# kureta/ddsp-pytorch

Hardware: AMD Instinct MI355X
Metric: audio samples/sec/GPU + %HBM-roofline, 16kHz/100-harmonic/batch512 (higher is better)
Workload: dtype f32

## Files before the change

ddsp-pytorch_amd/csrc/ddsp_osc.hip:

```cpp
#include <hip/hip_runtime.h>
#include <stdint.h>

#include <atomic>

#include "ddsp_hip.h"
#include "ddsp_internal.h"
#include "ddsp_osc_common.h"

using namespace ddsp_osc;

namespace {

template <int K, int MODE, bool POW2, int KL = K, int NS = 1, bool QREUSE = false>
__device__ __forceinline__ void walk_fast(const OscParams &p, FrameState<K> &st, int b, int t, int j, bool active,
                                          int i0, float L0, float L1, int n_beg, int n_end)
{
    extern __shared__ float ystage[];
    const float i0f = (float)i0;
    float *yframe = p.y + ((long)b * p.T + t) * p.R;
    float lam = 0.0f, dlam = 0.0f;
    if (POW2) {
        float w0s;
        upsample_weights(p.scale, t * p.R + n_beg, i0f, w0s, lam);
        dlam = (t == 0 && n_beg == 0) ? 0.0f : p.scale;
    }
#define DDSP_STAGE_END() __builtin_amdgcn_sched_barrier(0)
    constexpr bool QKEEP = QREUSE && (MODE == MODE_SYNTH) && POW2 && NS == 1;
    float qk[QKEEP ? KL : 1];
    auto one_step = [&](int n, const bool fresh) {
        float w0[NS], w1[NS];
#pragma unroll
        for (int e = 0; e < NS; ++e) {
            if (POW2) {
                w1[e] = lam;
                w0[e] = 1.0f - lam;
                lam += dlam;
            } else {
                upsample_weights(p.scale, t * p.R + n + e, i0f, w0[e], w1[e]);
            }
        }
// ... 452 lines not shown
    const double occupancy = K >= 20 ? 1.10 : (K >= 15 ? 1.03 : 1.0);
    const double waves = (double)(frames << logG) / 64.0;
    const double fill = waves >= 2048.0 ? 1.0 : (waves < 1.0 ? 1.0 : waves) / 2048.0;
    return waste * shared * occupancy / fill;
}

std::atomic<int> g_forced_k{0};
std::atomic<int> g_path{0};

bool pick_tiling(int H, long frames, Tiling *out)
{
    double best = 1e30;
    bool found = false;
    const int forced = g_forced_k.load(std::memory_order_relaxed);
    for (int K : kKs) {
        if (forced && K != forced) continue;
        const int lanes = (H + K - 1) / K;
        int logG = 0;
        while ((1 << logG) < lanes) ++logG;
        if (logG > 6) continue;
        const double cost = tiling_cost(H, K, logG, frames);
        if (cost < best) {
            best = cost;
            out->K = K;
            out->logG = logG;
            found = true;
        }
    }
    return found;
}

size_t frame_scratch_bytes(int B, int T, int H)
{
    const size_t n = (size_t)B * T * H;
    return 2 * align256(n * sizeof(float)) + align256(n * sizeof(double)) + align256(sup_elems(B, T, H) * sizeof(double)) + 256;
}

bool setup_params(OscParams &p, void *scratch, int B, int T, int H, int hop, int sample_rate)
{
    Tiling tl;
    if (!pick_tiling(H, (long)B * T, &tl)) return false;
    const size_t n = (size_t)B * T * H;
    char *base = (char *)scratch;
    p.w = (float *)base;
    p.amp = (float *)(base + align256(n * sizeof(float)));
    p.loc = (double *)(base + 2 * align256(n * sizeof(float)));
    p.sup = (double *)((char *)p.loc + align256(n * sizeof(double)));
    p.redo_flag = (int *)((char *)p.sup + align256(sup_elems(B, T, H) * sizeof(double)));
    p.B = B; p.T = T; p.H = H; p.R = hop;
    p.K = tl.K;
    p.logG = tl.logG;
    p.NSB = (T + (256 >> tl.logG) - 1) / (256 >> tl.logG);
    p.scale = (float)(1.0 / (double)hop);
    p.nyquist = (float)(sample_rate / 2);
    p.sr = (float)sample_rate;
    p.pow2 = ((hop & (hop - 1)) == 0 && hop >= 2 && (long)T * hop <= (1L << 23)) ? 1 : 0;
    p.stage_out = (p.pow2 && hop >= 64 && tl.logG >= 2 && tl.logG <= 4) ? 1 : 0;
    return true;
}

}

extern "C" int ddsp_osc_set_tiling(int harmonics_per_lane)
{
    if (harmonics_per_lane != 0) {
        if (!ddsp_hooks_on()) return DDSP_EPERM;
        bool known = false;
        for (int K : kKs) known = known || (K == harmonics_per_lane);
// ... 82 lines not shown
```

ddsp-pytorch_amd/csrc/ddsp_osc_chunk.hip:

```cpp
#include <hip/hip_runtime.h>
#include <stdint.h>

#include <atomic>
#include <mutex>
#include <stdlib.h>
#include <vector>

#include "ddsp_hip.h"
#include "ddsp_internal.h"
#include "ddsp_osc_common.h"
#include "ddsp_osc_plan.h"

#include <stddef.h>

using namespace ddsp_osc;

namespace {

#ifndef DDSP_TURN_EVERY
#define DDSP_TURN_EVERY 8
#endif
constexpr int kRow = 256 + 4;
constexpr float kReuseMaxInc = 4.8f;

#define DDSP_STAGE_END() __builtin_amdgcn_sched_barrier(0)

__device__ __forceinline__ void segment_lambda(const OscParams &p, int n, bool clamp0, float &lam, float &dlam)
{
    lam = clamp0 ? 0.0f : (float)(2 * n + 1) * p.inv2R;
    dlam = clamp0 ? 0.0f : 2.0f * p.inv2R;
}

__device__ __forceinline__ int wave_slot()
{
    return __builtin_amdgcn_s_getreg((4 << 0) | (0 << 6) | (3 << 11));
}
__device__ __forceinline__ void take_turn(int slot, int nres, int shift)
{
    const unsigned epoch = (unsigned)(__builtin_amdgcn_s_memrealtime() >> shift);
    const unsigned turn = epoch + (unsigned)slot;
    switch (nres >= 3 ? turn % 3u : (nres == 2 ? (turn & 1u) : 0u)) {
        case 0: __builtin_amdgcn_s_setprio(0); break;
        case 1: __builtin_amdgcn_s_setprio(1); break;
        default: __builtin_amdgcn_s_setprio(2); break;
    }
}

__device__ __forceinline__ float ldf(const float *base, unsigned idx)
{
    return *reinterpret_cast<const float *>(reinterpret_cast<const char *>(base) + (size_t)(idx * 4u));
}
__device__ __forceinline__ double ldd(const double *base, unsigned idx)
{
    return *reinterpret_cast<const double *>(reinterpret_cast<const char *>(base) + (size_t)(idx * 8u));
}

struct ChunkArgs {
    OscParams p;
    PlanTable t;
};
__device__ __forceinline__ const PlanTable *plan_table()
{
    return reinterpret_cast<const PlanTable *>((const char *)__builtin_amdgcn_kernarg_segment_ptr() + offsetof(ChunkArgs, t));
}

template <int K>
struct ParentTable {
    int v[kPlanMaxK];
    constexpr ParentTable() : v()
    {
        for (int d = 0; d < kPlanMaxK; ++d) v[d] = derived_parent(K, d);
    }
};
#define DDSP_PARENT(K, d) (par.v[d])

template <int K, int KR>
struct ChunkState {
    double acc[KR];
    float x0[KR], x1[KR];
    float a1[K], da[K];
};

struct Task {
    int wt, rb, c;
    int b, j;
    bool active;
    int i, i_end;
    int s, n;
};

__device__ __forceinline__ Task decode_task(const OscParams &p, int wt)
{
    Task k;
    k.wt = wt;
    k.rb = wt / p.NC;
    k.c = wt - k.rb * p.NC;
    const int lane = threadIdx.x & 63;
    k.j = lane & ((1 << p.logG) - 1);
    k.b = k.rb * (64 >> p.logG) + (lane >> p.logG);
    k.active = k.b < p.B;
    if (!k.active) k.b = p.B - 1;
    k.i = k.c * p.Lc;
    k.i_end = min(k.i + p.Lc, p.T * p.R);
    k.s = (k.i + (p.R >> 1)) >> p.lgR;
    k.n = (k.i + (p.R >> 1)) & (p.R - 1);
    return k;
}

__device__ __forceinline__ void segment_rows(int s, int T, int &r0, int &r1)
{
    r0 = s == 0 ? 0 : s - 1;
    r1 = s == 0 ? min(1, T - 1) : min(s, T - 1);
}

template <int K, int KR, int KLR, int NS, int QMODE>
__device__ __forceinline__ void walk_synth(const OscParams &p, ChunkState<K, KR> &st, const float (&fac)[K - KR + 1], float *ystage,
                                           float *yrow, int j, bool active, int i_abs, int n_beg, int n_end, bool clamp0, float L0,
                                           float L1, int slot)
{
    constexpr int KLD = KR < K ? class_derived(K, KLR) : 0;
    constexpr int KL = KLR + KLD;
#define DDSP_SLOT(m) ((m) < KLR ? (m) : KR + ((m) - KLR))
    constexpr ParentTable<K> par;
    const int G = 1 << p.logG, per = 32 >> p.logG;
    float lam, dlam;
    segment_lambda(p, n_beg, clamp0, lam, dlam);
    float mal = 1.0f - lam;
    float *ycol = ystage + threadIdx.x;
    const float *yblk = ystage + (threadIdx.x & ~(G - 1));
    static_assert(QMODE == 0 || (QMODE == 1 && NS == 1) || (QMODE == 2 && NS == 2), "quotient reuse: across iterations or inside a pair");
    float qk[QMODE == 1 ? KL : 1];
    constexpr int RUN = DDSP_TURN_EVERY < NS ? NS : DDSP_TURN_EVERY;
    for (int nb = n_beg; nb < n_end; nb += RUN) {
    take_turn(slot, p.nres, p.turn_shift);
    for (int n = nb; n < nb + RUN; n += NS) {
        float w0[NS], w1[NS];
        w1[0] = lam;
        w0[0] = mal;
#pragma unroll
        for (int e = 1; e < NS; ++e) {
            w1[e] = w1[e - 1] + dlam;
            w0[e] = w0[e - 1] - dlam;
        }
        float v[NS][KL];
        DDSP_STAGE_END();
#pragma unroll
        for (int e = 0; e < NS; ++e)
#pragma unroll
            for (int m = 0; m < KLR; ++m) v[e][m] = w1[e] * st.x1[m];
        DDSP_STAGE_END();
#pragma unroll
        for (int e = 0; e < NS; ++e)
#pragma unroll
            for (int m = 0; m < KLR; ++m) v[e][m] = __fmaf_rn(w0[e], st.x0[m], v[e][m]);
        DDSP_STAGE_END();
        double d[NS][KLR];
#pragma unroll
        for (int e = 0; e < NS; ++e)
#pragma unroll
            for (int m = 0; m < KLR; ++m) d[e][m] = (double)v[e][m];
        DDSP_STAGE_END();
#pragma unroll
        for (int e = 0; e < NS; ++e)
#pragma unroll
            for (int m = 0; m < KLR; ++m) {
                st.acc[m] += d[e][m];
                d[e][m] = st.acc[m];
// ... 155 lines not shown
    float lam, dlam;
    segment_lambda(p, n_beg, clamp0, lam, dlam);
    float mal = 1.0f - lam;
    for (int nb = n_beg; nb < n_end; nb += 16) {
    take_turn(slot, p.nres, p.turn_shift);
    for (int n = nb; n < nb + 16; ++n) {
        const float w1 = lam, w0 = mal;
        lam += dlam;
        mal -= dlam;
        float v[K];
        DDSP_STAGE_END();
#pragma unroll
        for (int m = 0; m < K; ++m) v[m] = w1 * x1[m];
        DDSP_STAGE_END();
#pragma unroll
        for (int m = 0; m < K; ++m) v[m] = __fmaf_rn(w0, x0[m], v[m]);
        DDSP_STAGE_END();
        double d[K];
#pragma unroll
        for (int m = 0; m < K; ++m) d[m] = (double)v[m];
        DDSP_STAGE_END();
#pragma unroll
        for (int m = 0; m < K; ++m) acc[m] += d[m];
        DDSP_STAGE_END();
    }
    }
}

__device__ __forceinline__ int group_max(int v, int logG)
{
    for (int o = 1; o < (1 << logG); o <<= 1) v = max(v, __shfl_xor(v, o));
    return v;
}

template <int K, int KR>
__global__ void __launch_bounds__(256, K <= 13 ? 3 : 1) osc_chunk_totals_kernel(ChunkArgs args)
{
    const OscParams &p = args.p;
    const int wt = blockIdx.x * 4 + __builtin_amdgcn_readfirstlane((int)(threadIdx.x >> 6));
    if (wt >= p.RB * p.NC) return;
    Task k = decode_task(p, wt);
    const int G = 1 << p.logG;
    const long rowbase = (long)k.b * p.T;
    const int i_beg = k.i;
    const int slot = wave_slot();
    int hs[K];
    {
        const PlanTable *tab = plan_table();
#pragma unroll
        for (int m = 0; m < K; ++m) hs[m] = tab->h[k.j * K + m];
    }
    int hmax = 0;

    auto make_row = [&](int r, float (&w)[KR]) {
        const float fb = p.f0[rowbase + r];
        const unsigned crow = ((unsigned)k.b * p.T + r) * p.H;
        float a0[K];
        float s = 0.0f;
#pragma unroll
        for (int m = 0; m < K; ++m) a0[m] = ldf(p.c, crow + min(hs[m], p.H - 1));
#pragma unroll
        for (int m = 0; m < K; ++m) {
            const int h = hs[m];
            const bool ok = h < p.H;
            const float hz = (float)(h + 1) * fb;
            a0[m] = (ok && !(hz > p.nyquist)) ? a0[m] : 0.0f;
            s += a0[m];
        }
        s = group_sum(s, p.logG);
        const float rs = 1.0f / s;
        const int seg_start = max(r * p.R - (p.R >> 1), 0);
        const bool own = k.active && seg_start >= i_beg && seg_start < k.i_end;
#pragma unroll
        for (int m = 0; m < K; ++m) {
            const int h = hs[m];
            const bool ok = h < p.H;
            const float wv = ok ? frame_increment(h, fb, p.sr) : 0.0f;
            if (m < KR) w[m < KR ? m : 0] = wv;
            const float amp = ok ? a0[m] * rs : 0.0f;
            if (amp != 0.0f) hmax = max(hmax, h + 1);
            if (ok && own) {
                p.w[crow + h] = wv;
                p.amp[crow + h] = amp;
            }
        }
    };

    float x0[KR], x1[KR];
    int r0, r1;
    segment_rows(k.s, p.T, r0, r1);
    make_row(r0, x0);
    make_row(r1, x1);
    double acc[KR];
#pragma unroll
    for (int m = 0; m < KR; ++m) acc[m] = 0.0;
    while (true) {
        const int n_end = min(p.R, k.n + (k.i_end - k.i));
        walk_totals<KR>(p, acc, x0, x1, k.n, n_end, k.s == 0, slot);
        k.i += n_end - k.n;
        if (k.i >= k.i_end) break;
        ++k.s; k.n = 0;
        if (k.s >= 2) {
#pragma unroll
            for (int m = 0; m < KR; ++m) x0[m] = x1[m];
            if (k.s <= p.T - 1) make_row(k.s, x1);
        }
    }
    hmax = group_max(hmax, p.logG);
    if (k.active) {
        double *cp = p.ctot + ((long)k.b * p.NC + k.c) * p.HC + k.j;
#pragma unroll
        for (int m = 0; m < KR; ++m)
            if (hs[m] < p.H) cp[m * G] = acc[m];
        if (k.j == 0) p.rlive[(long)k.b * p.NC + k.c] = hmax;
    }
}

__global__ void __launch_bounds__(512) osc_chunk_scan_kernel(OscParams p, int nscan_blocks, int Q)
{
    __shared__ double seg_tot[8][64];
    const int lane = threadIdx.x & 63, q = threadIdx.x >> 6;
    if (blockIdx.x == 0 && threadIdx.x == 0) {
        *p.redo_flag = 0;
        p.frame_flag[2] = 0;
    }
    if ((int)blockIdx.x < nscan_blocks) {
        const long ncol = (long)p.B * p.HC;
        const long idx = (long)blockIdx.x * 64 + lane;
        const bool live = idx < ncol && q < Q;
        const int b = live ? (int)(idx / p.HC) : 0, h = live ? (int)(idx - (long)b * p.HC) : 0;
        double *col = p.ctot + (long)b * p.NC * p.HC + h;
        const int per = (p.NC + Q - 1) / Q, c_beg = q * per, c_end = min(c_beg + per, p.NC);
        if (per <= 32) {
            double v[32];
            double tot = 0.0;
#pragma unroll
            for (int i = 0; i < 32; ++i) {
                v[i] = (live && c_beg + i < c_end) ? col[(long)(c_beg + i) * p.HC] : 0.0;
                tot += v[i];
            }
// ... 39 lines not shown
        return;
    }
    const long wv = (long)(blockIdx.x - nscan_blocks) * (blockDim.x >> 6) + q;
    const int c = (int)wv;
    if (c >= p.NC) return;
    const int Bpad = p.RB * (64 >> p.logG);
    int *out = p.perm + (long)c * Bpad;
    auto cls_of = [&](int ml) {
        if (ml < 0) return -1;
        int q = 0;
        while (q < 4 && ml <= p.cls_max[q]) ++q;
        return q;
    };
    int base[5], cnt[5] = {0, 0, 0, 0, 0};
    for (int b0 = 0; b0 < p.B; b0 += 64) {
        const int b = b0 + lane;
        const int cls = cls_of(b < p.B ? p.rlive[(long)b * p.NC + c] : -1);
        for (int q = 0; q < 5; ++q) cnt[q] += __popcll(__ballot(cls == q));
    }
    base[0] = 0;
    for (int q = 1; q < 5; ++q) base[q] = base[q - 1] + cnt[q - 1];
    for (int b0 = 0; b0 < p.B; b0 += 64) {
        const int b = b0 + lane;
        const int cls = cls_of(b < p.B ? p.rlive[(long)b * p.NC + c] : -1);
        for (int q = 0; q < 5; ++q) {
            const unsigned long long mask = __ballot(cls == q);
            if (cls == q) out[base[q] + __popcll(mask & ((1ull << lane) - 1ull))] = b;
            base[q] += __popcll(mask);
        }
    }
    for (int b = p.B + lane; b < Bpad; b += 64) out[b] = -1;
}

#ifdef DDSP_CHUNK_STAMPS
__device__ long g_stamps[16384 * 4];
extern "C" int ddsp_osc_read_stamps(long *host, int ntasks)
{
    return (int)hipMemcpyFromSymbol(host, HIP_SYMBOL(g_stamps), sizeof(long) * 4 * (size_t)(ntasks < 16384 ? ntasks : 16384));
}
#endif

#ifndef DDSP_CHUNK_INLINE_REPAIR
#define DDSP_CHUNK_INLINE_REPAIR 1
#endif
template <int K, int KR, bool EXACT>
__global__ void __launch_bounds__(256, (!EXACT && K <= 13) ? 3 : 1) osc_chunk_synth_kernel(ChunkArgs args)
{
    const OscParams &p = args.p;
    extern __shared__ float ystage[];
    constexpr int KD = K - KR;
    constexpr ParentTable<K> par;
    constexpr int KE = class_prefix(KR, 3), KQ = class_prefix(KR, 2), KH = class_prefix(KR, 1), KT = class_prefix(KR, 0);
    const int ntasks = p.RB * p.NC;
    const PlanTable *tab = plan_table();
    const int jj = (threadIdx.x & 63) & ((1 << p.logG) - 1);
    float fac[KD + 1];
#pragma unroll
    for (int d = 0; d < KD; ++d) fac[d] = (float)(1u << tab->shift[jj * K + KR + d]);
    fac[KD] = 1.0f;
    int wt = blockIdx.x * 4 + __builtin_amdgcn_readfirstlane((int)(threadIdx.x >> 6));
    if (EXACT && *p.redo_flag == 0) return;
    for (; wt < ntasks; wt += gridDim.x * 4) {
        if (EXACT && p.redo[wt] == 0) continue;
#ifdef DDSP_CHUNK_STAMPS
        const long stamp0 = wall_clock64();
#endif
        if (!EXACT && wt == 0 && (threadIdx.x & 63) == 0) clock_stamp(p.redo_flag, 0);
        bool exact = EXACT;
      for (;;) {
        Task k = decode_task(p, wt);
        {
            const int idx = k.rb * (64 >> p.logG) + ((threadIdx.x & 63) >> p.logG);
            const int b = p.perm[(long)k.c * (p.RB * (64 >> p.logG)) + idx];
            k.active = b >= 0;
            k.b = k.active ? b : p.perm[(long)k.c * (p.RB * (64 >> p.logG))];
        }
        const int G = 1 << p.logG;
        const long rowbase = (long)k.b * p.T;
        float *yrow = p.y + (long)k.b * p.T * p.R;
        ChunkState<K, KR> st;
        const int slot = exact ? 0 : wave_slot();
        bool bad = false;
        const unsigned cbase = ((unsigned)k.b * p.NC + k.c) * p.HC + k.j;
#pragma unroll
        for (int m = 0; m < KR; ++m) {
            const double v = ldd(p.ctot, cbase + (unsigned)(m * G));
            st.acc[m] = (tab->h[k.j * K + m] < p.H) ? v : 0.0;
            bad = bad || !(st.acc[m] >= 0.0);
        }
        int mlive = p.H;
        if (!exact) {
            mlive = p.rlive[(long)k.b * p.NC + k.c];
#pragma unroll
            for (int o = 32; o > 0; o >>= 1) mlive = max(mlive, __shfl_xor(mlive, o));
            mlive = __builtin_amdgcn_readfirstlane(mlive);
        }
        int r0, r1;
        segment_rows(k.s, p.T, r0, r1);
        float L0, L1;
        auto load_rows = [&](int ra, int rb2, bool first) {
            const unsigned o0 = ((unsigned)k.b * p.T + ra) * p.H, o1 = ((unsigned)k.b * p.T + rb2) * p.H;
            float t0[KR], t1[KR], u0[K], u1[K];
            int hs[K];
#pragma unroll
            for (int m = 0; m < K; ++m) hs[m] = tab->h[k.j * K + m];
#pragma unroll
            for (int m = 0; m < K; ++m) {
                const unsigned g = (unsigned)min(hs[m], p.H - 1);
                if (m < KR) {
                    t0[m < KR ? m : 0] = first ? ldf(p.w, o0 + g) : 0.0f;
                    t1[m < KR ? m : 0] = ldf(p.w, o1 + g);
                }
                u0[m] = first ? ldf(p.amp, o0 + g) : 0.0f;
                u1[m] = ldf(p.amp, o1 + g);
            }
#pragma unroll
            for (int m = 0; m < K; ++m) {
                const bool ok = hs[m] < p.H;
                if (m < KR) {
                    if (first) st.x0[m < KR ? m : 0] = ok ? t0[m < KR ? m : 0] : 0.0f;
                    st.x1[m < KR ? m : 0] = ok ? t1[m < KR ? m : 0] : 0.0f;
                }
                const float older = first ? (ok ? u0[m] : 0.0f) : st.a1[m];
                st.a1[m] = ok ? u1[m] : 0.0f;
                st.da[m] = st.a1[m] - older;
            }
            if (first) L0 = p.a[rowbase + ra]; else L0 = L1;
            L1 = p.a[rowbase + rb2];
        };
        load_rows(r0, r1, true);
#ifdef DDSP_CHUNK_STAMPS
        long stamp_walk = 0;
        if (DDSP_CHUNK_STAMPS == 2) {
            float chk = 0.0f;
#pragma unroll
            for (int m = 0; m < KR; ++m) chk += st.x1[m] + st.da[m];
            if (__any(chk == 123456.0f)) bad = true;
            stamp_walk = wall_clock64();
        }
#endif
        while (true) {
            const int n_end = min(p.R, k.n + (k.i_end - k.i));
            const bool clamp0 = k.s == 0;
            bool big = false;
#pragma unroll
            for (int m = 0; m < KR; ++m) {
                bad = bad || !(st.x0[m] >= 0.0f) || !(st.x1[m] >= 0.0f);
                big = big || !(st.x0[m] < kReuseMaxInc) || !(st.x1[m] < kReuseMaxInc);
            }
#pragma unroll
            for (int d = 0; d < KD; ++d)
                big = big || !(fac[d] * st.x0[DDSP_PARENT(K, d)] < kReuseMaxInc) || !(fac[d] * st.x1[DDSP_PARENT(K, d)] < kReuseMaxInc);
            if (exact) {
                walk_synth_exact<K, KR>(p, st, fac, yrow, k.j, k.active, k.i, k.n, n_end, clamp0, L0, L1);
            } else if (mlive <= p.cls_max[3] && KE < KQ) {
                walk_synth<K, KR, KE, 4, 0>(p, st, fac, ystage, yrow, k.j, k.active, k.i, k.n, n_end, clamp0, L0, L1, slot);
            } else if (mlive <= p.cls_max[2] && KQ < KH) {
                walk_synth<K, KR, KQ, 4, 0>(p, st, fac, ystage, yrow, k.j, k.active, k.i, k.n, n_end, clamp0, L0, L1, slot);
            } else if (mlive <= p.cls_max[1] && KH < KT) {
                walk_synth<K, KR, KH, 2, 0>(p, st, fac, ystage, yrow, k.j, k.active, k.i, k.n, n_end, clamp0, L0, L1, slot);
            } else if (mlive <= p.cls_max[0] && KT < KR) {
                walk_synth<K, KR, KT, 1, 0>(p, st, fac, ystage, yrow, k.j, k.active, k.i, k.n, n_end, clamp0, L0, L1, slot);
            } else if (!__any(big)) {
                walk_synth<K, KR, KR, 1, 1>(p, st, fac, ystage, yrow, k.j, k.active, k.i, k.n, n_end, clamp0, L0, L1, slot);
            } else {
                walk_synth<K, KR, KR, 1, 0>(p, st, fac, ystage, yrow, k.j, k.active, k.i, k.n, n_end, clamp0, L0, L1, slot);
            }
            k.i += n_end - k.n;
            if (k.i >= k.i_end) break;
            ++k.s; k.n = 0;
            if (k.s >= 2) {
#pragma unroll
                for (int m = 0; m < KR; ++m) st.x0[m] = st.x1[m];
                segment_rows(k.s, p.T, r0, r1);
                load_rows(r0, r1, false);
            }
        }
        if (!exact) {
#pragma unroll
            for (int m = 0; m < KR; ++m) bad = bad || !(st.acc[m] < (double)kFastPhaseLimit);
#pragma unroll
            for (int d = 0; d < KD; ++d) bad = bad || !((double)fac[d] * st.acc[DDSP_PARENT(K, d)] < (double)kFastPhaseLimit);
            const bool redo = __any(bad);
            if (DDSP_CHUNK_INLINE_REPAIR && redo) { exact = true; continue; }
            if ((threadIdx.x & 63) == 0) {
                p.redo[wt] = redo ? 1 : 0;
                if (redo) atomicOr(p.redo_flag, 1);
                if (wt == 0) clock_stamp(p.redo_flag, 1);
            }
#ifdef DDSP_CHUNK_STAMPS
            if ((threadIdx.x & 63) == 0 && wt < 16384) {
                g_stamps[wt * 4 + 0] = stamp0;
                g_stamps[wt * 4 + 1] = wall_clock64();
                g_stamps[wt * 4 + 2] = __builtin_amdgcn_s_getreg((4 << 0) | (0 << 6) | (31 << 11));
                g_stamps[wt * 4 + 3] = DDSP_CHUNK_STAMPS == 2 ? stamp_walk : (long)__builtin_amdgcn_s_getreg((20 << 0) | (0 << 6) | (31 << 11));
            }
#endif
        } else if (DDSP_CHUNK_INLINE_REPAIR && !EXACT && (threadIdx.x & 63) == 0) {
            p.redo[wt] = 0;
            if (wt == 0) clock_stamp(p.redo_flag, 1);
        }
        break;
      }
    }
}

struct Residency { int cus, wg_per_cu; };

template <int K, int KR>
hipError_t synth_residency(Residency *out)
{
    static std::mutex mu;
    static Residency cache[64] = {};
    int dev = 0;
    hipError_t e = hipGetDevice(&dev);
    if (e != hipSuccess) return e;
    dev &= 63;
    std::lock_guard<std::mutex> lk(mu);
    if (cache[dev].cus == 0) {
        int cus = 0, nb = 0;
        e = hipDeviceGetAttribute(&cus, hipDeviceAttributeMultiprocessorCount, dev);
        if (e != hipSuccess) return e;
        e = hipOccupancyMaxActiveBlocksPerMultiprocessor(&nb, osc_chunk_synth_kernel<K, KR, false>, 256, sizeof(float) * 32 * kRow);
        if (e != hipSuccess) return e;
        if (cus <= 0 || nb <= 0) return hipErrorInvalidValue;
        cache[dev].cus = cus;
        cache[dev].wg_per_cu = nb;
// ... 40 lines not shown
        long Lc = (N + nc - 1) / nc;
        Lc = (Lc + 31) & ~31L;
        if (Lc < R) Lc = R;
        if (Lc == lastLc) continue;
        lastLc = (int)Lc;
        const long NC = (N + Lc - 1) / Lc;
        const long wgs = (NC * RB + 3) / 4;
        const long per_cu = (wgs + cus - 1) / cus;
        const double alone = per_cu == 1 ? 1.9 : (per_cu == 2 ? 1.03 : 1.0);
        const double cost = (double)per_cu * alone * ((double)Lc + c0);
        if (cost < best) {
            best = cost;
            bestLc = (int)Lc;
            bestNC = (int)NC;
        }
        if (Lc == R) break;
    }
    (void)wg_per_cu;
    *Lc_out = bestLc;
    *NC_out = bestNC;
}

bool chunked_eligible(const OscParams &p)
{
    if (!(p.pow2 && p.R >= 64 && p.R <= 8192 && p.logG >= 2 && p.logG <= 4 && !p.live_in && !p.live_out && !p.dbg_phi &&
          (long)p.B * p.T * p.H < (1L << 29)))
        return false;
    const int gpw = 64 >> p.logG, rb = (p.B + gpw - 1) / gpw;
    return (long)p.B * 100 >= (long)rb * gpw * 88 || g_chunk_any_batch.load(std::memory_order_relaxed);
}

size_t chunk_scratch_bytes(int B, int T, int H)
{
    return frame_scratch_bytes(B, T, H) + 2 * align256((size_t)B * T * sizeof(int)) +
           align256((size_t)T * ((size_t)B + 16) * sizeof(int)) + 256;
}

template <int K>
hipError_t chunk_geometry(OscParams &p, Residency *res_out)
{
    Residency res;
    const SlotPlan &pl = slot_plan(p.H, K, 1 << p.logG);
    hipError_t e = pl.KD ? synth_residency<K, plan_roots(K)>(&res) : synth_residency<K, K>(&res);
    if (e != hipSuccess) return e;
    p.HC = pl.KD ? pl.KR << p.logG : p.H;
    for (int q = 0; q < 4; ++q) p.cls_max[q] = pl.cls_max[q];
    const int GPW = 64 >> p.logG;
    p.RB = (p.B + GPW - 1) / GPW;
    p.lgR = 0;
    while ((1 << p.lgR) < p.R) ++p.lgR;
    p.inv2R = 0.5f / (float)p.R;
    pick_chunks(p.T, p.R, p.RB, res.cus, res.wg_per_cu, &p.Lc, &p.NC);
    if (ddsp_hooks_on()) {
        const char *e = getenv("DDSP_OSC_CHUNK_LEN");
        const int v = e ? atoi(e) : 0;
        if (v >= p.R && v % 32 == 0) {
            p.Lc = v;
            p.NC = (int)(((long)p.T * p.R + v - 1) / v);
        }
    }
    p.nres = res.wg_per_cu < 3 ? (res.wg_per_cu < 1 ? 1 : res.wg_per_cu) : 3;
    {
        const double ticks = (double)p.Lc * (double)p.K * 5.6;
        int sh = 8;
        while (sh < 16 && (double)(1 << (sh + 1)) <= ticks / 6.0) ++sh;
        p.turn_shift = sh;
        if (ddsp_hooks_on()) {
            const char *e = getenv("DDSP_OSC_TURN_SHIFT");
            const int v = e ? atoi(e) : 0;
            if (v >= 6 && v <= 20) p.turn_shift = v;
        }
    }
    *res_out = res;
    return hipSuccess;
}

void carve_chunk_scratch(OscParams &p, void *scratch)
{
    const size_t n = (size_t)p.B * p.T * p.H;
    char *base = (char *)scratch;
    p.frame_flag = p.redo_flag;
    p.w = (float *)base;
    p.amp = (float *)(base + align256(n * sizeof(float)));
    p.ctot = (double *)(base + 2 * align256(n * sizeof(float)));
    p.rlive = (int *)(base + frame_scratch_bytes(p.B, p.T, p.H));
    p.perm = (int *)((char *)p.rlive + align256((size_t)p.B * p.NC * sizeof(int)));
    p.redo = (int *)((char *)p.perm + align256((size_t)p.NC * p.RB * (64 >> p.logG) * sizeof(int)));
    p.redo_flag = (int *)((char *)p.redo + align256((size_t)p.RB * p.NC * sizeof(int)));
}

template <int K, int KR>
hipError_t launch_plan(const OscParams &p, const SlotPlan &pl, hipStream_t s)
{
    ChunkArgs args;
    args.p = p;
    args.t = pl.t;
    const long tasks = (long)p.RB * p.NC;
    const unsigned grid = (unsigned)((tasks + 3) / 4);
    int slot = ddsp_prof::begin(ddsp_prof::TOTALS, s);
    hipLaunchKernelGGL((osc_chunk_totals_kernel<K, KR>), dim3(grid), dim3(256), 0, s, args);
    ddsp_prof::end(slot, s);
    slot = ddsp_prof::begin(ddsp_prof::SCAN, s);
    const long nscan_blocks = ((long)p.B * p.HC + 63) / 64;
    const int Q = p.NC > 128 ? 8 : (p.NC > 64 ? 4 : (p.NC > 32 ? 2 : 1));
    hipLaunchKernelGGL(osc_chunk_scan_kernel, dim3((unsigned)(nscan_blocks + (p.NC + Q - 1) / Q)), dim3(64 * Q), 0, s, p, (int)nscan_blocks, Q);
    ddsp_prof::end(slot, s);
    slot = ddsp_prof::begin(ddsp_prof::SYNTH, s);
    hipLaunchKernelGGL((osc_chunk_synth_kernel<K, KR, false>), dim3(grid), dim3(256), sizeof(float) * 32 * kRow, s, args);
    ddsp_prof::end(slot, s);
    if (!DDSP_CHUNK_INLINE_REPAIR) {
        const unsigned rgrid = grid < 256u ? grid : 256u;
        hipLaunchKernelGGL((osc_chunk_synth_kernel<K, KR, true>), dim3(rgrid), dim3(256), 0, s, args);
    }
    return hipGetLastError();
}

template <int K>
hipError_t launch_chunked(OscParams p, void *scratch, hipStream_t s)
{
    Residency res;
    hipError_t e = chunk_geometry<K>(p, &res);
    if (e != hipSuccess) return e;
    carve_chunk_scratch(p, scratch);
    const SlotPlan &pl = slot_plan(p.H, K, 1 << p.logG);
    return pl.KD ? launch_plan<K, plan_roots(K)>(p, pl, s) : launch_plan<K, K>(p, pl, s);
}

hipError_t chunk_geometry_k(OscParams &p, int *cus, int *wg_per_cu)
{
    Residency res = {};
    hipError_t e = hipErrorInvalidValue;
    switch (p.K) {
#define DDSP_CASE(KK) case KK: e = chunk_geometry<KK>(p, &res); break;
        DDSP_CASE(4) DDSP_CASE(8) DDSP_CASE(12) DDSP_CASE(13) DDSP_CASE(15) DDSP_CASE(16) DDSP_CASE(20) DDSP_CASE(23) DDSP_CASE(25)
#undef DDSP_CASE
        default: break;
    }
    *cus = res.cus;
    *wg_per_cu = res.wg_per_cu;
    return e;
}

const int *chunk_flag_words(OscParams p)
{
    int cus = 0, wgs = 0;
    if (chunk_geometry_k(p, &cus, &wgs) != hipSuccess) return p.redo_flag;
    carve_chunk_scratch(p, (void *)p.w);
    return p.redo_flag;
}

hipError_t launch_chunked_k(const OscParams &p, void *scratch, hipStream_t s)
{
    switch (p.K) {
#define DDSP_CASE(KK) case KK: return launch_chunked<KK>(p, scratch, s);
        DDSP_CASE(4) DDSP_CASE(8) DDSP_CASE(12) DDSP_CASE(13) DDSP_CASE(15) DDSP_CASE(16) DDSP_CASE(20) DDSP_CASE(23) DDSP_CASE(25)
#undef DDSP_CASE
// ... 6 lines not shown
```

ddsp-pytorch_amd/csrc/ddsp_osc_common.h:

```cpp
#pragma once
#include <hip/hip_runtime.h>
#include <stdint.h>

#include <atomic>

namespace ddsp_osc {


constexpr float kTwoPi32 = 6.2831854820251465f;
constexpr float kInvTwoPi32 = 0.15915493667125702f;
constexpr float kRevPerRad = 0.15915494309189535f;
constexpr float kFastPhaseLimit = 1.0e7f;
constexpr float kRoundMagic = 12582912.0f;
constexpr int kFrameScratchTag = 0x46524d45;

struct OscParams {
    const float *f0, *c, *a;
    float *y;
    float *w, *amp;
    double *loc;
    double *sup;
    int *redo_flag;
    const float *live_in;
    float *live_out;
    float *dbg_phi;
    const float *grad_y;
    float *part_c;
    float *part_a;
    float *grad_c, *grad_a;
    int B, T, H, R;
    int K;
    int logG;
    int NSB;
    int force_exact;
    int stage_out;
    int pow2;
    double *ctot;
    int *rlive;
    int *perm;
    int *redo;
    int *frame_flag;
    int Lc, NC, RB;
    int HC;
    int cls_max[4];
    int lgR;
    int nres;
    int turn_shift;
    float inv2R;
    float scale;
    float nyquist;
    float sr;
};

__device__ __forceinline__ unsigned xcd_block(unsigned bid, unsigned nblocks)
{
    const unsigned per = nblocks >> 3;
    if (per == 0 || bid >= (per << 3)) return bid;
    return (bid & 7u) * per + (bid >> 3);
}

__device__ __forceinline__ void clock_stamp(int *redo_flag, int which)
{
    unsigned long long *w = reinterpret_cast<unsigned long long *>(redo_flag + 16) + 2 * which;
    w[0] = __builtin_amdgcn_s_memtime();
    w[1] = __builtin_amdgcn_s_memrealtime();
}

template <int CTRL>
__device__ __forceinline__ float dpp_mov(float v)
// ... 99 lines not shown
```

ddsp-pytorch_amd/csrc/ddsp_osc_plan.h:

```cpp
#pragma once
#include <stdint.h>

#include <algorithm>
#include <set>
#include <vector>

namespace ddsp_osc {

constexpr int kPlanMaxLanes = 16, kPlanMaxK = 25, kPlanMaxSlots = kPlanMaxLanes * kPlanMaxK;
constexpr int kPlanParents = 7;
constexpr int kPlanMaxChildren = 3;
constexpr uint16_t kNoHarmonic = 0xffff;

constexpr int pick7(int i, int a, int b, int c, int d, int e, int f, int g)
{
    return i == 0 ? a : i == 1 ? b : i == 2 ? c : i == 3 ? d : i == 4 ? e : i == 5 ? f : i == 6 ? g : 0;
}
constexpr int slot_children(int K, int i)
{
    switch (K) {
        case 4: return pick7(i, 1, 0, 0, 0, 0, 0, 0);
        case 8: return pick7(i, 2, 1, 0, 0, 0, 0, 0);
        case 12: return pick7(i, 3, 2, 1, 0, 0, 0, 0);
        case 13: return pick7(i, 3, 2, 1, 0, 0, 0, 0);
        case 15: return pick7(i, 3, 2, 1, 1, 0, 0, 0);
        case 16: return pick7(i, 3, 2, 1, 1, 0, 0, 0);
        case 20: return pick7(i, 3, 2, 2, 1, 1, 0, 0);
        case 23: return pick7(i, 3, 2, 2, 1, 1, 1, 0);
        case 25: return pick7(i, 3, 2, 2, 1, 1, 1, 1);
        default: return 0;
    }
}
constexpr int plan_derived(int K)
// ... 123 lines not shown
    if (!s.place(0)) return false;

    pl.H = H; pl.K = K; pl.G = G; pl.KR = KR; pl.KD = KD;
    for (int i = 0; i < kPlanMaxSlots; ++i) { pl.t.h[i] = kNoHarmonic; pl.t.shift[i] = 0; }
    int derived = 0;
    for (int sz = kPlanMaxChildren + 1; sz >= 1; --sz) {
        std::vector<const Piece *> ps;
        for (const Piece &p : s.pieces)
            if (p.size_class == sz) ps.push_back(&p);
        std::sort(ps.begin(), ps.end(), [](const Piece *a, const Piece *b) { return a->members[0] < b->members[0]; });
        std::vector<int> idx;
        for (int i = 0; i < KR; ++i)
            if (1 + slot_children(K, i) == sz) idx.push_back(i);
        for (size_t n = 0; n < ps.size(); ++n) {
            const int i = idx[n / G], j = (int)(n % G);
            const std::vector<int> &mem = ps[n]->members;
            pl.t.h[j * K + i] = (uint16_t)(mem[0] - 1);
            for (size_t c = 1; c < mem.size(); ++c) {
                int d = 0;
                while (!(derived_parent(K, d) == i && derived_rank(K, d) == (int)c - 1)) ++d;
                int t = 0;
                while ((mem[0] << t) < mem[c]) ++t;
                pl.t.h[j * K + KR + d] = (uint16_t)(mem[c] - 1);
                pl.t.shift[j * K + KR + d] = (uint8_t)t;
                ++derived;
            }
        }
    }
    if (derived < 1) return false;
    plan_class_limits(pl);
    return true;
}

}
```

Baseline: 28.53 billion.

## Pack per-lane frame records contiguously and prefetch next row ahead of walks

Replaces the separate per-harmonic w and amp scratch arrays with one packed per-lane record of increments and amplitudes, written and read as float4 vectors. The synth kernel then loads rows with contiguous vector loads instead of scattered per-harmonic loads. The totals kernel now issues the next row's f0 and coefficient loads before walking the current segment so their latency overlaps compute, and the synth walk touches the next record early as a prefetch. Scratch layout and sizing are reworked to fit the record buffer, and debug stamp instrumentation is extended under an ifdef.

```diff
diff --git a/ddsp-pytorch_amd/csrc/ddsp_osc.hip b/ddsp-pytorch_amd/csrc/ddsp_osc.hip
--- a/ddsp-pytorch_amd/csrc/ddsp_osc.hip
+++ b/ddsp-pytorch_amd/csrc/ddsp_osc.hip
@@ -6,6 +6,7 @@
 #include "ddsp_hip.h"
 #include "ddsp_internal.h"
 #include "ddsp_osc_common.h"
+#include "ddsp_osc_plan.h"
 
 using namespace ddsp_osc;
 
@@ -524,8 +525,7 @@
 
 size_t frame_scratch_bytes(int B, int T, int H)
 {
-    const size_t n = (size_t)B * T * H;
-    return 2 * align256(n * sizeof(float)) + align256(n * sizeof(double)) + align256(sup_elems(B, T, H) * sizeof(double)) + 256;
+    return frame_layout_bytes((size_t)B, (size_t)T, (size_t)H);
 }
 
 bool setup_params(OscParams &p, void *scratch, int B, int T, int H, int hop, int sample_rate)
diff --git a/ddsp-pytorch_amd/csrc/ddsp_osc_chunk.hip b/ddsp-pytorch_amd/csrc/ddsp_osc_chunk.hip
--- a/ddsp-pytorch_amd/csrc/ddsp_osc_chunk.hip
+++ b/ddsp-pytorch_amd/csrc/ddsp_osc_chunk.hip
@@ -53,6 +53,25 @@
 __device__ __forceinline__ double ldd(const double *base, unsigned idx)
 {
     return *reinterpret_cast<const double *>(reinterpret_cast<const char *>(base) + (size_t)(idx * 8u));
+}
+
+#ifndef DDSP_ROWS_AHEAD_TOTALS
+#define DDSP_ROWS_AHEAD_TOTALS 1
+#endif
+#ifndef DDSP_ROWS_AHEAD_SYNTH
+#define DDSP_ROWS_AHEAD_SYNTH 1
+#endif
+
+template <int K, int KR>
+__device__ __forceinline__ float4 *record_ptr(float *rec, int b, int T, int r, int logG, int j)
+{
+    return reinterpret_cast<float4 *>(rec) + ((((size_t)b * (size_t)T + (size_t)r) << logG) + (size_t)j) * (size_t)(record_floats(K, KR) / 4);
+}
+template <int N>
+__device__ __forceinline__ float &record_at(float4 (&v)[N], int i)
+{
+    float4 &t = v[i >> 2];
+    return (i & 3) == 0 ? t.x : (i & 3) == 1 ? t.y : (i & 3) == 2 ? t.z : t.w;
 }
 
 struct ChunkArgs {
@@ -116,7 +135,7 @@
 template <int K, int KR, int KLR, int NS, int QMODE>
 __device__ __forceinline__ void walk_synth(const OscParams &p, ChunkState<K, KR> &st, const float (&fac)[K - KR + 1], float *ystage,
                                            float *yrow, int j, bool active, int i_abs, int n_beg, int n_end, bool clamp0, float L0,
-                                           float L1, int slot)
+                                           float L1, int slot, bool touch, unsigned touch_rec, float &ahead)
 {
     constexpr int KLD = KR < K ? class_derived(K, KLR) : 0;
     constexpr int KL = KLR + KLD;
@@ -133,6 +152,8 @@
     constexpr int RUN = DDSP_TURN_EVERY < NS ? NS : DDSP_TURN_EVERY;
     for (int nb = n_beg; nb < n_end; nb += RUN) {
     take_turn(slot, p.nres, p.turn_shift);
+    if (DDSP_ROWS_AHEAD_SYNTH && touch && nb == n_beg)
+        ahead = *reinterpret_cast<const float *>(reinterpret_cast<const float4 *>(p.rec) + (size_t)touch_rec * (size_t)(record_floats(K, KR) / 4));
     for (int n = nb; n < nb + RUN; n += NS) {
         float w0[NS], w1[NS];
         w1[0] = lam;
@@ -354,6 +375,45 @@
     for (int o = 1; o < (1 << logG); o <<= 1) v = max(v, __shfl_xor(v, o));
     return v;
 }
+
+#ifdef DDSP_CHUNK_STAMPS
+__device__ long g_stamps[16384 * 4];
+extern "C" int ddsp_osc_read_stamps(long *host, int ntasks)
+{
+    return (int)hipMemcpyFromSymbol(host, HIP_SYMBOL(g_stamps), sizeof(long) * 4 * (size_t)(ntasks < 16384 ? ntasks : 16384));
+}
+constexpr int kMidCrossing = 5;
+__device__ long g_xstamps[2][16384 * 8];
+extern "C" int ddsp_osc_read_row_stamps(long *host, int ntasks, int which)
+{
+    return (int)hipMemcpyFromSymbol(host, HIP_SYMBOL(g_xstamps), sizeof(long) * 8 * (size_t)(ntasks < 16384 ? ntasks : 16384),
+                                    sizeof(long) * 8 * 16384 * (size_t)(which ? 1 : 0));
+}
+struct CrossStamps {
+    long start, sum, mid, c0;
+    int cnt;
+    __device__ __forceinline__ void begin() { start = wall_clock64(); sum = 0; mid = 0; cnt = 0; }
+    __device__ __forceinline__ void enter() { c0 = (long)__builtin_amdgcn_s_memtime(); }
+    __device__ __forceinline__ void leave()
+    {
+        sum += (long)__builtin_amdgcn_s_memtime() - c0;
+        if (++cnt == kMidCrossing) mid = wall_clock64();
+    }
+    __device__ __forceinline__ void write(int which, int wt)
+    {
+        if ((threadIdx.x & 63) != 0 || wt >= 16384) return;
+        long *o = g_xstamps[which] + (size_t)wt * 8;
+        o[0] = start;
+        o[1] = wall_clock64();
+        o[2] = __builtin_amdgcn_s_getreg((4 << 0) | (0 << 6) | (31 << 11));
+        o[3] = __builtin_amdgcn_s_getreg((20 << 0) | (0 << 6) | (31 << 11));
+        o[4] = sum;
+        o[5] = cnt;
+        o[6] = mid;
+        o[7] = 0;
+    }
+};
+#endif
 
 template <int K, int KR>
 __global__ void __launch_bounds__(256, K <= 13 ? 3 : 1) osc_chunk_totals_kernel(ChunkArgs args)
@@ -374,13 +434,15 @@
     }
     int hmax = 0;
 
-    auto make_row = [&](int r, float (&w)[KR]) {
-        const float fb = p.f0[rowbase + r];
+    constexpr int RECF = record_floats(K, KR);
+    auto fetch_row = [&](int r, float &fb, float (&a0)[K]) {
+        fb = p.f0[rowbase + r];
         const unsigned crow = ((unsigned)k.b * p.T + r) * p.H;
-        float a0[K];
+#pragma unroll
+        for (int m = 0; m < K; ++m) a0[m] = ldf(p.c, crow + min(hs[m], p.H - 1));
+    };
+    auto finish_row = [&](int r, float fb, float (&a0)[K], float (&w)[KR]) {
         float s = 0.0f;
-#pragma unroll
-        for (int m = 0; m < K; ++m) a0[m] = ldf(p.c, crow + min(hs[m], p.H - 1));
 #pragma unroll
         for (int m = 0; m < K; ++m) {
             const int h = hs[m];
@@ -393,41 +455,83 @@
         const float rs = 1.0f / s;
         const int seg_start = max(r * p.R - (p.R >> 1), 0);
         const bool own = k.active && seg_start >= i_beg && seg_start < k.i_end;
+        float4 rec[RECF / 4];
+#pragma unroll
+        for (int i = KR + K; i < RECF; ++i) record_at(rec, i) = 0.0f;
 #pragma unroll
         for (int m = 0; m < K; ++m) {
             const int h = hs[m];
             const bool ok = h < p.H;
-            const float wv = ok ? frame_increment(h, fb, p.sr) : 0.0f;
-            if (m < KR) w[m < KR ? m : 0] = wv;
+            if (m < KR) {
+                const float wv = ok ? frame_increment(h, fb, p.sr) : 0.0f;
+                w[m < KR ? m : 0] = wv;
+                record_at(rec, record_inc_slot(m < KR ? m : 0)) = wv;
+            }
             const float amp = ok ? a0[m] * rs : 0.0f;
             if (amp != 0.0f) hmax = max(hmax, h + 1);
-            if (ok && own) {
-                p.w[crow + h] = wv;
-                p.amp[crow + h] = amp;
-            }
+            record_at(rec, record_amp_slot(KR, m)) = amp;
+        }
+        if (own) {
+            float4 *dst = record_ptr<K, KR>(p.rec, k.b, p.T, r, p.logG, k.j);
+#pragma unroll
+            for (int q = 0; q < RECF / 4; ++q) dst[q] = rec[q];
         }
     };
 
     float x0[KR], x1[KR];
+    float fbn, cn[K];
     int r0, r1;
     segment_rows(k.s, p.T, r0, r1);
-    make_row(r0, x0);
-    make_row(r1, x1);
+    fetch_row(r0, fbn, cn);
+    finish_row(r0, fbn, cn, x0);
+    fetch_row(r1, fbn, cn);
+    finish_row(r1, fbn, cn, x1);
     double acc[KR];
 #pragma unroll
     for (int m = 0; m < KR; ++m) acc[m] = 0.0;
+#ifdef DDSP_CHUNK_STAMPS
+    CrossStamps xs;
+    xs.begin();
+#endif
     while (true) {
         const int n_end = min(p.R, k.n + (k.i_end - k.i));
-        walk_totals<KR>(p, acc, x0, x1, k.n, n_end, k.s == 0, slot);
-        k.i += n_end - k.n;
-        if (k.i >= k.i_end) break;
-        ++k.s; k.n = 0;
-        if (k.s >= 2) {
+        const int sn = k.s + 1;
+        const bool makes = sn >= 2 && sn <= p.T - 1;
+        if (DDSP_ROWS_AHEAD_TOTALS && makes && k.i + (n_end - k.n) < k.i_end) {
+            fetch_row(sn, fbn, cn);
+            walk_totals<KR>(p, acc, x0, x1, k.n, n_end, k.s == 0, slot);
+            k.i += n_end - k.n;
+            k.s = sn; k.n = 0;
+#ifdef DDSP_CHUNK_STAMPS
+            xs.enter();
+#endif
 #pragma unroll
             for (int m = 0; m < KR; ++m) x0[m] = x1[m];
-            if (k.s <= p.T - 1) make_row(k.s, x1);
-        }
-    }
+            finish_row(sn, fbn, cn, x1);
+        } else {
+            walk_totals<KR>(p, acc, x0, x1, k.n, n_end, k.s == 0, slot);
+            k.i += n_end - k.n;
+            if (k.i >= k.i_end) break;
+            k.s = sn; k.n = 0;
+            if (sn < 2) continue;
+#ifdef DDSP_CHUNK_STAMPS
+            xs.enter();
+#endif
+#pragma unroll
+            for (int m = 0; m < KR; ++m) x0[m] = x1[m];
+            if (makes) {
+                fetch_row(sn, fbn, cn);
+                finish_row(sn, fbn, cn, x1);
+            }
+        }
+#ifdef DDSP_CHUNK_STAMPS
+        if (__any(x1[KR - 1] == 123456.0f)) hmax = p.H;
+        xs.leave();
+#endif
+    }
+#ifdef DDSP_CHUNK_STAMPS
+    xs.write(0, wt);
+#endif
     hmax = group_max(hmax, p.logG);
     if (k.active) {
         double *cp = p.ctot + ((long)k.b * p.NC + k.c) * p.HC + k.j;
@@ -533,14 +637,6 @@
     for (int b = p.B + lane; b < Bpad; b += 64) out[b] = -1;
 }
 
-#ifdef DDSP_CHUNK_STAMPS
-__device__ long g_stamps[16384 * 4];
-extern "C" int ddsp_osc_read_stamps(long *host, int ntasks)
-{
-    return (int)hipMemcpyFromSymbol(host, HIP_SYMBOL(g_stamps), sizeof(long) * 4 * (size_t)(ntasks < 16384 ? ntasks : 16384));
-}
-#endif
-
 #ifndef DDSP_CHUNK_INLINE_REPAIR
 #define DDSP_CHUNK_INLINE_REPAIR 1
 #endif
@@ -565,6 +661,8 @@
         if (EXACT && p.redo[wt] == 0) continue;
 #ifdef DDSP_CHUNK_STAMPS
         const long stamp0 = wall_clock64();
+        CrossStamps xs;
+        xs.begin();
 #endif
         if (!EXACT && wt == 0 && (threadIdx.x & 63) == 0) clock_stamp(p.redo_flag, 0);
         bool exact = EXACT;
@@ -599,31 +697,25 @@
         int r0, r1;
         segment_rows(k.s, p.T, r0, r1);
         float L0, L1;
+        constexpr int RQ = record_floats(K, KR) / 4;
         auto load_rows = [&](int ra, int rb2, bool first) {
-            const unsigned o0 = ((unsigned)k.b * p.T + ra) * p.H, o1 = ((unsigned)k.b * p.T + rb2) * p.H;
-            float t0[KR], t1[KR], u0[K], u1[K];
-            int hs[K];
-#pragma unroll
-            for (int m = 0; m < K; ++m) hs[m] = tab->h[k.j * K + m];
+            const float4 *q1 = record_ptr<K, KR>(p.rec, k.b, p.T, rb2, p.logG, k.j);
+            const float4 *q0 = record_ptr<K, KR>(p.rec, k.b, p.T, ra, p.logG, k.j);
+            float4 v0[RQ], v1[RQ];
+#pragma unroll
+            for (int q = 0; q < RQ; ++q) {
+                if (first) v0[q] = q0[q];
+                v1[q] = q1[q];
+            }
+#pragma unroll
+            for (int m = 0; m < KR; ++m) {
+                if (first) st.x0[m] = record_at(v0, record_inc_slot(m));
+                st.x1[m] = record_at(v1, record_inc_slot(m));
+            }
 #pragma unroll
             for (int m = 0; m < K; ++m) {
-                const unsigned g = (unsigned)min(hs[m], p.H - 1);
-                if (m < KR) {
-                    t0[m < KR ? m : 0] = first ? ldf(p.w, o0 + g) : 0.0f;
-                    t1[m < KR ? m : 0] = ldf(p.w, o1 + g);
-                }
-                u0[m] = first ? ldf(p.amp, o0 + g) : 0.0f;
-                u1[m] = ldf(p.amp, o1 + g);
-            }
-#pragma unroll
-            for (int m = 0; m < K; ++m) {
-                const bool ok = hs[m] < p.H;
-                if (m < KR) {
-                    if (first) st.x0[m < KR ? m : 0] = ok ? t0[m < KR ? m : 0] : 0.0f;
-                    st.x1[m < KR ? m : 0] = ok ? t1[m < KR ? m : 0] : 0.0f;
-                }
-                const float older = first ? (ok ? u0[m] : 0.0f) : st.a1[m];
-                st.a1[m] = ok ? u1[m] : 0.0f;
+                const float older = first ? record_at(v0, record_amp_slot(KR, m)) : st.a1[m];
+                st.a1[m] = record_at(v1, record_amp_slot(KR, m));
                 st.da[m] = st.a1[m] - older;
             }
             if (first) L0 = p.a[rowbase + ra]; else L0 = L1;
@@ -643,6 +735,9 @@
         while (true) {
             const int n_end = min(p.R, k.n + (k.i_end - k.i));
             const bool clamp0 = k.s == 0;
+            const bool more = k.i + (n_end - k.n) < k.i_end;
+            const unsigned touch_rec = (((unsigned)k.b * p.T + (unsigned)min(k.s + 1, p.T - 1)) << p.logG) + (unsigned)k.j;
+            float ahead = 0.0f;
             bool big = false;
 #pragma unroll
             for (int m = 0; m < KR; ++m) {
@@ -655,26 +750,44 @@
             if (exact) {
                 walk_synth_exact<K, KR>(p, st, fac, yrow, k.j, k.active, k.i, k.n, n_end, clamp0, L0, L1);
             } else if (mlive <= p.cls_max[3] && KE < KQ) {
-                walk_synth<K, KR, KE, 4, 0>(p, st, fac, ystage, yrow, k.j, k.active, k.i, k.n, n_end, clamp0, L0, L1, slot);
+                walk_synth<K, KR, KE, 4, 0>(p, st, fac, ystage, yrow, k.j, k.active, k.i, k.n, n_end, clamp0, L0, L1, slot, more, touch_rec, ahead);
             } else if (mlive <= p.cls_max[2] && KQ < KH) {
-                walk_synth<K, KR, KQ, 4, 0>(p, st, fac, ystage, yrow, k.j, k.active, k.i, k.n, n_end, clamp0, L0, L1, slot);
+                walk_synth<K, KR, KQ, 4, 0>(p, st, fac, ystage, yrow, k.j, k.active, k.i, k.n, n_end, clamp0, L0, L1, slot, more, touch_rec, ahead);
             } else if (mlive <= p.cls_max[1] && KH < KT) {
-                walk_synth<K, KR, KH, 2, 0>(p, st, fac, ystage, yrow, k.j, k.active, k.i, k.n, n_end, clamp0, L0, L1, slot);
+                walk_synth<K, KR, KH, 2, 0>(p, st, fac, ystage, yrow, k.j, k.active, k.i, k.n, n_end, clamp0, L0, L1, slot, more, touch_rec, ahead);
             } else if (mlive <= p.cls_max[0] && KT < KR) {
-                walk_synth<K, KR, KT, 1, 0>(p, st, fac, ystage, yrow, k.j, k.active, k.i, k.n, n_end, clamp0, L0, L1, slot);
+                walk_synth<K, KR, KT, 1, 0>(p, st, fac, ystage, yrow, k.j, k.active, k.i, k.n, n_end, clamp0, L0, L1, slot, more, touch_rec, ahead);
             } else if (!__any(big)) {
-                walk_synth<K, KR, KR, 1, 1>(p, st, fac, ystage, yrow, k.j, k.active, k.i, k.n, n_end, clamp0, L0, L1, slot);
+                walk_synth<K, KR, KR, 1, 1>(p, st, fac, ystage, yrow, k.j, k.active, k.i, k.n, n_end, clamp0, L0, L1, slot, more, touch_rec, ahead);
             } else {
-                walk_synth<K, KR, KR, 1, 0>(p, st, fac, ystage, yrow, k.j, k.active, k.i, k.n, n_end, clamp0, L0, L1, slot);
+                walk_synth<K, KR, KR, 1, 0>(p, st, fac, ystage, yrow, k.j, k.active, k.i, k.n, n_end, clamp0, L0, L1, slot, more, touch_rec, ahead);
             }
             k.i += n_end - k.n;
+            if (DDSP_ROWS_AHEAD_SYNTH) {
+                asm volatile("" : "+v"(ahead));
+                bad = bad || !(ahead >= 0.0f);
+            }
             if (k.i >= k.i_end) break;
             ++k.s; k.n = 0;
             if (k.s >= 2) {
+#ifdef DDSP_CHUNK_STAMPS
+                xs.enter();
+#endif
 #pragma unroll
                 for (int m = 0; m < KR; ++m) st.x0[m] = st.x1[m];
                 segment_rows(k.s, p.T, r0, r1);
                 load_rows(r0, r1, false);
+#ifdef DDSP_CHUNK_STAMPS
+                {
+                    float chk = 0.0f;
+#pragma unroll
+                    for (int m = 0; m < KR; ++m) chk += st.x1[m];
+#pragma unroll
+                    for (int m = 0; m < K; ++m) chk += st.da[m];
+                    if (__any(chk == 123456.0f)) bad = true;
+                }
+                xs.leave();
+#endif
             }
         }
         if (!exact) {
@@ -694,6 +807,7 @@
                 g_stamps[wt * 4 + 0] = stamp0;
                 g_stamps[wt * 4 + 1] = wall_clock64();
                 g_stamps[wt * 4 + 2] = __builtin_amdgcn_s_getreg((4 << 0) | (0 << 6) | (31 << 11));
+                xs.write(1, wt);
                 g_stamps[wt * 4 + 3] = DDSP_CHUNK_STAMPS == 2 ? stamp_walk : (long)__builtin_amdgcn_s_getreg((20 << 0) | (0 << 6) | (31 << 11));
             }
 #endif
@@ -800,8 +914,11 @@
 
 size_t chunk_scratch_bytes(int B, int T, int H)
 {
-    return frame_scratch_bytes(B, T, H) + 2 * align256((size_t)B * T * sizeof(int)) +
-           align256((size_t)T * ((size_t)B + 16) * sizeof(int)) + 256;
+    size_t bytes = frame_scratch_bytes(B, T, H) + chunk_small_bytes((size_t)B, (size_t)T);
+    Tiling tl;
+    if (pick_tiling(H, (long)B * T, &tl) && tl.logG >= 2 && tl.logG <= 4)
+        bytes += chunk_tail_bytes((size_t)B, (size_t)T, (size_t)H, tl.K, 1 << tl.logG);
+    return bytes;
 }
 
 template <int K>
@@ -843,18 +960,19 @@
     return hipSuccess;
 }
 
-void carve_chunk_scratch(OscParams &p, void *scratch)
-{
-    const size_t n = (size_t)p.B * p.T * p.H;
+bool carve_chunk_scratch(OscParams &p, void *scratch)
+{
+    const SlotPlan &pl = slot_plan(p.H, p.K, 1 << p.logG);
+    const ChunkLayout l = chunk_layout((size_t)p.B, (size_t)p.T, (size_t)p.H, p.K, pl.KR, 1 << p.logG, (size_t)p.NC, (size_t)p.HC);
     char *base = (char *)scratch;
     p.frame_flag = p.redo_flag;
-    p.w = (float *)base;
-    p.amp = (float *)(base + align256(n * sizeof(float)));
-    p.ctot = (double *)(base + 2 * align256(n * sizeof(float)));
-    p.rlive = (int *)(base + frame_scratch_bytes(p.B, p.T, p.H));
+    p.rec = (float *)base;
+    p.ctot = (double *)(base + l.ctot_off);
+    p.rlive = (int *)(base + l.small_off);
     p.perm = (int *)((char *)p.rlive + align256((size_t)p.B * p.NC * sizeof(int)));
     p.redo = (int *)((char *)p.perm + align256((size_t)p.NC * p.RB * (64 >> p.logG) * sizeof(int)));
     p.redo_flag = (int *)((char *)p.redo + align256((size_t)p.RB * p.NC * sizeof(int)));
+    return l.ok;
 }
 
 template <int K, int KR>
@@ -889,7 +1007,7 @@
     Residency res;
     hipError_t e = chunk_geometry<K>(p, &res);
     if (e != hipSuccess) return e;
-    carve_chunk_scratch(p, scratch);
+    if (!carve_chunk_scratch(p, scratch)) return hipErrorInvalidValue;
     const SlotPlan &pl = slot_plan(p.H, K, 1 << p.logG);
     return pl.KD ? launch_plan<K, plan_roots(K)>(p, pl, s) : launch_plan<K, K>(p, pl, s);
 }
diff --git a/ddsp-pytorch_amd/csrc/ddsp_osc_common.h b/ddsp-pytorch_amd/csrc/ddsp_osc_common.h
--- a/ddsp-pytorch_amd/csrc/ddsp_osc_common.h
+++ b/ddsp-pytorch_amd/csrc/ddsp_osc_common.h
@@ -35,6 +35,7 @@
     int force_exact;
     int stage_out;
     int pow2;
+    float *rec;
     double *ctot;
     int *rlive;
     int *perm;
diff --git a/ddsp-pytorch_amd/csrc/ddsp_osc_plan.h b/ddsp-pytorch_amd/csrc/ddsp_osc_plan.h
--- a/ddsp-pytorch_amd/csrc/ddsp_osc_plan.h
+++ b/ddsp-pytorch_amd/csrc/ddsp_osc_plan.h
@@ -1,4 +1,5 @@
 #pragma once
+#include <stddef.h>
 #include <stdint.h>
 
 #include <algorithm>
@@ -188,4 +189,48 @@
     return true;
 }
 
-}
+constexpr int record_floats(int K, int KR) { return (KR + K + 3) & ~3; }
+constexpr size_t record_base(size_t b, size_t T, size_t r, int G, int j, int K, int KR)
+{
+    return ((b * T + r) * (size_t)G + (size_t)j) * (size_t)record_floats(K, KR);
+}
+constexpr int record_inc_slot(int m) { return m; }
+constexpr int record_amp_slot(int KR, int m) { return KR + m; }
+
+inline size_t plan_align256(size_t n) { return (n + 255) & ~(size_t)255; }
+inline size_t frame_layout_bytes(size_t B, size_t T, size_t H)
+{
+    const size_t n = B * T * H;
+    return 2 * plan_align256(n * 4) + plan_align256(n * 8) + plan_align256(B * ((T + 3) / 4) * H * 8) + 256;
+}
+inline size_t chunk_small_bytes(size_t B, size_t T)
+{
+    return 2 * plan_align256(B * T * 4) + plan_align256(T * (B + 16) * 4) + 256;
+}
+struct ChunkLayout {
+    size_t rec_bytes, ctot_off, ctot_bytes, small_off, end;
+    bool ok;
+};
+inline ChunkLayout chunk_layout(size_t B, size_t T, size_t H, int K, int KR, int G, size_t NC, size_t HC)
+{
+    ChunkLayout l;
+    const size_t flag_off = frame_layout_bytes(B, T, H) - 256;
+    l.rec_bytes = plan_align256(B * T * (size_t)G * (size_t)record_floats(K, KR) * 4);
+    l.ctot_bytes = plan_align256(B * NC * HC * 8);
+    l.small_off = flag_off + 256;
+    l.ctot_off = std::max(2 * plan_align256(B * T * H * 4), l.rec_bytes);
+    l.end = l.small_off + chunk_small_bytes(B, T);
+    l.ok = l.rec_bytes <= flag_off;
+    if (l.ctot_off + l.ctot_bytes > flag_off) {
+        l.ctot_off = l.end;
+        l.end += l.ctot_bytes;
+    }
+    return l;
+}
+inline size_t chunk_tail_bytes(size_t B, size_t T, size_t H, int K, int G)
+{
+    const ChunkLayout l = chunk_layout(B, T, H, K, K, G, T, H);
+    return l.end - (frame_layout_bytes(B, T, H) + chunk_small_bytes(B, T));
+}
+
+}
```

Result: no change. 28.55 billion (median of 6 runs) (+0.1%).
